# Open-Sentra/beatrice

Measured on AMD Instinct MI355X. Metric: Mpps + achieved HBM GB/s, device-resident parse+filter, 64B and IMIX, higher is better.
Workload: dtype u8; 1 GPU; C2 frames + filter: 16M x 64B Eth/IPv4/UDP, fixed stride, parse + PacketFilter (udp, 10.x.x.x/8, 1000-2000) + ordered compaction (metric's 64B parse+filter); packets_per_gpu=16777216, packets_total=16777216, parallelism=batch split x1, devices_distinct=1, rehearsal_one_device=False

## Files before the change

beatrice_amd/csrc/bt_context.cpp:

```cpp
#include <sched.h>
#include <sys/syscall.h>
#include <unistd.h>

#include <algorithm>
#include <cctype>
#include <cstdarg>
#include <cstdio>
#include <cstdlib>
#include <cstring>
#include <functional>
#include <mutex>
#include <string>
#include <thread>

#include "bt_ctx.h"
#include "bt_hip_util.h"

using namespace bt;

namespace {

thread_local std::string g_err;

}
// ... 213 lines not shown
uint32_t bt_usable_cpus(void) { return bt::usable_cpus(); }

void bt_destroy(bt_ctx* c) {
    const bt::DeviceRestore keep_device;
    if (!c) return;
    (void)hipSetDevice(c->device);
    (void)hipDeviceSynchronize();
    for (const auto& r : c->host_regs)
        (void)bt::pin_release(reinterpret_cast<const void*>(r.first), r.second);
    c->host_regs.clear();
    release_host_pipe(c);
    if (c->pcap) { bt::pcap_stage_free(c->pcap); c->pcap = nullptr; }
    c->pool.reset();
    release_timing_graph(c);
    release_workspace(c);
    release_dfa_pools(c);
    release_timing(c);
    release_extract_stage(c);
    release_xfer(c);
    release_walk_stages(c);
    if (c->stream) (void)hipStreamDestroy(c->stream);
    delete c;
}

int bt_host_parallel(bt_ctx* c, void (*fn)(void*, uint32_t, uint32_t), void* user) {
    if (!c || !fn) return set_error(BT_E_INVALID_ARGUMENT, "null argument");
    bt::host_parallel(c, [&](unsigned w, unsigned T) { fn(user, w, T); });
    return BT_OK;
}

int bt_stream_create(bt_ctx* c, void** stream) {
    const bt::DeviceRestore keep_device;
    if (!c || !stream) return set_error(BT_E_INVALID_ARGUMENT, "null argument");
    HIP_TRY(hipSetDevice(c->device));
    hipStream_t s = nullptr;
    HIP_TRY(hipStreamCreateWithFlags(&s, hipStreamNonBlocking));
    *stream = s;
    return BT_OK;
}

int bt_stream_synchronize(bt_ctx* c, void* stream) {
    const bt::DeviceRestore keep_device;
    if (!c || !stream) return set_error(BT_E_INVALID_ARGUMENT, "null argument");
    HIP_TRY(hipSetDevice(c->device));
    HIP_TRY(hipStreamSynchronize(reinterpret_cast<hipStream_t>(stream)));
    return BT_OK;
}

int bt_stream_destroy(bt_ctx* c, void* stream) {
    const bt::DeviceRestore keep_device;
    if (!c || !stream) return set_error(BT_E_INVALID_ARGUMENT, "null argument");
    HIP_TRY(hipSetDevice(c->device));
    HIP_TRY(hipStreamSynchronize(reinterpret_cast<hipStream_t>(stream)));
    HIP_TRY(hipStreamDestroy(reinterpret_cast<hipStream_t>(stream)));
    return BT_OK;
}

int bt_synchronize(bt_ctx* c) {
    const bt::DeviceRestore keep_device;
    if (!c) return set_error(BT_E_INVALID_ARGUMENT, "null context");
    HIP_TRY(hipSetDevice(c->device));
    HIP_TRY(hipStreamSynchronize(c->stream));
    if (c->ws.cstream) HIP_TRY(hipStreamSynchronize(c->ws.cstream));
    return BT_OK;
}

}

namespace bt {

int ctx_device(const bt_ctx* c) { return c->device; }

bool ctx_stream_busy(bt_ctx* c) {
    const bt::DeviceRestore keep_device;
    if (hipSetDevice(c->device) != hipSuccess) return false;
    return hipStreamQuery(c->stream) == hipErrorNotReady;
}

}
```

beatrice_amd/csrc/bt_ctx.h:

```cpp
#pragma once

#include <hip/hip_runtime.h>
#include <sched.h>

#include <atomic>
#include <chrono>
#include <cstdlib>
#include <memory>
#include <mutex>
#include <utility>
#include <vector>

#include "beatrice_gpu_bench.h"
#include "bt_device.h"
#include "bt_pack.h"
#include "bt_tally.h"
#include "bt_fanout.h"
#include "bt_flowtab.h"
#include "bt_host_pool.h"
#include "bt_host.h"

#define HIP_TRY(x)                                                                       \
    do {                                                                                 \
        hipError_t e_ = (x);                                                             \
// ... 17 lines not shown
    uint8_t* d_in = nullptr;
    uint8_t* h_out = nullptr;
    uint8_t* d_out = nullptr;
    uint32_t* d_tile = nullptr;
    bool busy = false;
    uint32_t lo = 0, cnt = 0;
};

struct PcapStage;
void pcap_stage_free(PcapStage* s);

}

struct bt_ctx {
    int device = 0;
    hipStream_t stream = nullptr;
    bt_opts opts{};
    int grid = 0;
    std::mutex mu;
    int spin_rc = -1;
    unsigned device_flags = 0;

    std::vector<bt_filter_slot> slots;
    bt::DevProgram prog{};
    std::vector<uint8_t> dfa_pool;
    std::atomic<uint32_t> staged_window[2] = {{0u}, {0u}};
    struct DfaPools {
        uint8_t* dev[2] = {nullptr, nullptr};
        std::vector<std::pair<hipStream_t, hipEvent_t>> readers[2];
        std::vector<hipEvent_t> spare;
        int cur = 0;
    } dfa;

    struct Ws {
        uint32_t* chunk_sums = nullptr;
        uint64_t* verdict = nullptr;
        bt::PackChunkSum* pack_sums = nullptr;
        bt::TallyPartial* tally_parts = nullptr;
        uint8_t* fan_parts = nullptr;
        uint8_t* fan_queue = nullptr;
        hipStream_t last = nullptr;
        bool lazy = false;
        hipEvent_t sync = nullptr;
    };
    static constexpr int kMainDone = 8;
    struct Workspace {
        uint32_t cap = 0;
        Ws buf[2];
        int next = 0;
        hipEvent_t main_done[kMainDone] = {};
        int md_next = 0;
        hipStream_t cstream = nullptr;
    } ws;
    const void* last_base = nullptr;
    bool last_base_host = false;

    struct WalkStage {
        bt::RingBlock* h = nullptr;
        uint32_t cap = 0;
        hipEvent_t done = nullptr;
        bool used = false;
    };
    struct WalkStages {
        WalkStage stage[2];
        int next = 0;
    } walk;

    struct HostPipe {
        uint32_t chunk = 0;
        bt::HostSlot hs[2];
        bool ready = false;
        std::atomic<int> waiters{0};
        uint64_t last_caller = 0;
        uint64_t last_end = 0;
        bool shared_call = false;
    } host;
    std::unique_ptr<bt::HostPool> pool;
    std::once_flag pool_once;
    int numa_node = -1;
    cpu_set_t pin{};
    bool pinned = false;

    struct Timing {
        hipEvent_t ev0 = nullptr, ev1 = nullptr;
        hipEvent_t pipe_done = nullptr;
        hipEvent_t pipe_step = nullptr;
        std::vector<hipEvent_t> tev;
    } timing;
    struct TimingGraph {
        hipGraphExec_t exec = nullptr;
        bt_batch batch{};
        bt_outputs out{};
        uint32_t iters = 0;
    } tgraph;

    std::vector<std::pair<uintptr_t, uint64_t>> host_regs;

    struct Xfer {
        std::mutex mu;
        uint8_t* h[2] = {nullptr, nullptr};
        hipEvent_t ev[2] = {nullptr, nullptr};
        hipEvent_t after = nullptr;
    } xfer;

    struct ExtractStage {
        uint8_t* h = nullptr;
        uint8_t* d = nullptr;
        size_t cap = 0;
    } ex;

    bt::PcapStage* pcap = nullptr;
};

namespace bt {

void release_host_pipe(bt_ctx* c);
void release_timing_graph(bt_ctx* c);
void release_workspace(bt_ctx* c);
void release_dfa_pools(bt_ctx* c);
void release_timing(bt_ctx* c);
void release_extract_stage(bt_ctx* c);
void release_xfer(bt_ctx* c);
void release_walk_stages(bt_ctx* c);

HostPool& pool_of(bt_ctx* c);

int dfa_read_on(bt_ctx* c, hipStream_t st);

int ensure_ws(bt_ctx* c, uint32_t n);
int take_ws(bt_ctx* c, uint32_t n, bt_ctx::Ws** w);
int ws_touch(bt_ctx* c, bt_ctx::Ws* w, hipStream_t s);
int ws_done(bt_ctx* c, bt_ctx::Ws* w, hipStream_t s);
int ensure_cstream(bt_ctx* c);
bool host_resident(bt_ctx* c, const void* base);
int check_bounds(hipStream_t st, hipStream_t cst, const char* what);
int run_device(bt_ctx* c, const bt_batch* b, const bt_outputs* o, hipStream_t st, bool aos,
               hipEvent_t e0, hipEvent_t e1, hipStream_t cst = nullptr, hipEvent_t done = nullptr);
int run_pass_pack(bt_ctx* c, const bt_batch* b, const uint64_t* select, const bt_pack_opts* po,
                  const bt_pack_out* out, hipStream_t st, hipEvent_t e0, hipEvent_t e1);

int run_tally(bt_ctx* c, const uint8_t* decide, uint32_t n, const bt_batch* frames, const void* records, uint32_t n_cap,
              uint32_t flags, bt_tally* out, hipStream_t st, hipEvent_t e0, hipEvent_t e1);

int run_fanout(bt_ctx* c, const bt_batch* frames, const uint64_t* select, const bt_fanout_opts* opts, const bt_fanout_out* out,
               hipStream_t st, hipEvent_t e0, hipEvent_t e1);

int run_flow_table(bt_ctx* c, const bt_batch* frames, const uint64_t* select, const bt_flow_table_opts* opts, void* scratch,
                   uint64_t scratch_bytes, const bt_flow_table_out* out, hipStream_t st, hipEvent_t e0, hipEvent_t e1);

int run_flow_track_update(bt_ctx* c, void* state, const bt_batch* frames, const uint64_t* select, const bt_flow_track_update* upd,
                          void* scratch, uint64_t scratch_bytes, const bt_flow_track_out* out, hipStream_t st, hipEvent_t e0,
                          hipEvent_t e1);

int run_flow_tcp(bt_ctx* c, const bt_batch* frames, const uint32_t* flow_id, uint32_t table_flags, bt_flow_tcp_rec* tcp,
                 uint32_t flow_cap, bt_flow_tcp_result* result, hipStream_t st, hipEvent_t e0, hipEvent_t e1);

int run_flow_track_top(bt_ctx* c, const void* state, const bt_flow_top_opts* opts, const bt_flow_tcp_rec* tcp, void* scratch,
                       uint64_t scratch_bytes, const bt_flow_top_out* out, hipStream_t st, hipEvent_t e0, hipEvent_t e1);

int run_flow_track_hosts(bt_ctx* c, const void* state, const bt_flow_hosts_opts* opts, const bt_flow_tcp_rec* tcp, void* scratch,
                         uint64_t scratch_bytes, const bt_flow_hosts_out* out, hipStream_t st, hipEvent_t e0, hipEvent_t e1);

int build_table(const bt_field_def* f, uint32_t n, ExTable* t, uint64_t* span_out, bool* never);
int run_extract(bt_ctx* c, const bt_batch* b, const ExTable& t, bool never, const bt_extract_out* o, hipStream_t st,
                hipEvent_t e0 = nullptr, hipEvent_t e1 = nullptr);

unsigned pipeline_share(const bt_ctx* c);
void publish_staged_window(bt_ctx* c);

template <class Fn>
void pipeline_run(bt_ctx* c, uint32_t cnt, unsigned T, Fn&& fn) {
// ... 41 lines not shown
```

beatrice_amd/csrc/bt_device.h:

```cpp
#pragma once

#include <stdint.h>

#include "beatrice_gpu.h"
#include "bt_bounds.h"
#include "bt_frames.h"

namespace bt {

struct DevFilter {
    uint32_t kind, a, b, ctl;
    uint32_t mask, lo, span, pad;
};
constexpr uint32_t kSelIp = 0, kSelPort = 1, kSelProto = 2, kSelPbit = 3;
constexpr uint32_t kGateNone = 0, kGateIpv4 = 1, kGateL4 = 2;
constexpr uint32_t kResPred = 0, kResThrow = 1, kResHost = 2;

struct DevProgram {
    uint32_t n;
    uint32_t pad[3];
    DevFilter f[BT_MAX_FILTERS];
};

struct MainArgs : FrameSrc {
    uint32_t n_cap;
    uint8_t* records;
    uint8_t* decide;
    uint64_t* verdict;
    uint32_t blocked;
    uint32_t nt;
    const uint8_t* dfa;
    uint32_t dfa_bytes;
    uint32_t prefixes;
    uint32_t lean;
    uint32_t lean_lo;
};
constexpr uint32_t kLeanPcie = 38;
constexpr uint32_t kLeanLo = 12;

constexpr uint32_t kDfaPoolMax = 16384;

constexpr int kWave = 64;
constexpr int kWavesPerBlock = 4;
constexpr int kBlock = kWave * kWavesPerBlock;
constexpr int kRowDwords = 33;
constexpr int kChunkTiles = 256;
constexpr uint32_t kNeedParse = 102;
constexpr uint32_t kNeedFilter = 38;

enum RecLayout { kRecNone = 0, kRecPlanes = 1, kRecAoS = 2, kRecTiled = 3 };
int launch_main(const MainArgs& a, const DevProgram& prog, int rec_layout, bool filter,
                int grid_blocks, bool prefetch, void* stream, void* timing_start = nullptr,
                void* timing_stop = nullptr);
int launch_compact(const uint64_t* verdict, uint32_t n, uint32_t* chunk_sums, uint32_t* pass_idx,
                   uint32_t* n_pass, void* stream);

struct ResumeArgs : FrameSrc {
    uint8_t* decide;
    const uint8_t* dfa;
    uint32_t dfa_bytes;
};
int launch_payload_resume(const ResumeArgs& a, const DevProgram& prog, void* stream, void* timing_start = nullptr,
                          void* timing_stop = nullptr);
int launch_verdict_words(const uint8_t* decide, uint32_t n, uint64_t* verdict, void* stream);
uint32_t bounds_take_resume(void* stream, BoundsLog* first);

inline uint64_t read_limit(const void* base, uint64_t bytes) {
    const uint64_t b = (uint64_t)(uintptr_t)base;
    return bytes ? ((b + bytes + 15u) & ~15ull) - b : 0u;
}

uint32_t bounds_take_main(void* stream, BoundsLog* first);
uint32_t bounds_take_extract(void* stream, BoundsLog* first);

struct RingBlock {
    uint32_t block;
    uint32_t n;
    uint32_t start;
    uint32_t first_off;
};
struct RingWalkArgs {
    const uint8_t* ring;
    uint64_t block_size;
    const RingBlock* blocks;
    uint32_t count;
    bt_pkt_desc* desc;
    uint32_t cap;
    uint32_t* bad;
};
int launch_ring_walk(const RingWalkArgs& a, void* stream);
uint32_t bounds_take_ring(void* stream, BoundsLog* first);

constexpr uint32_t kExWindow = 256;
struct ExField {
    uint32_t offset, length;
    uint32_t ctl;
    uint32_t pad;
};
struct ExTable {
    uint32_t n;
    uint32_t span;
    uint32_t window;
    uint32_t row_dw;
    ExField f[BT_FIELD_MAX];
};
struct ExArgs : FrameSrc {
// ... 14 lines not shown
```

beatrice_amd/csrc/bt_kernels.hip:

```cpp
#include <algorithm>
#include <cstdlib>
#include <type_traits>

#include "bt_dev_util.h"
#include "bt_device.h"
#include "bt_hip_launch.h"
#include "bt_payload_walk.h"
#include "bt_slot_eval.h"

namespace bt {

__device__ BoundsLog g_bounds_main;

namespace {

__device__ __forceinline__ uint32_t be32_of(const uint32_t* w, int i) {
    return (byte_of(w, i) << 24) | (byte_of(w, i + 1) << 16) | (byte_of(w, i + 2) << 8) | byte_of(w, i + 3);
}

__device__ __forceinline__ bool is_vlan(uint32_t et) { return et == 0x8100u || et == 0x88A8u; }

__device__ __forceinline__ uint4 ld16(const uint8_t* p, bool nt) {
    if (nt) {
        const u32x4 x = __builtin_nontemporal_load(reinterpret_cast<const u32x4*>(p));
        return make_uint4(x.x, x.y, x.z, x.w);
    }
    return *reinterpret_cast<const uint4*>(p);
}
__device__ __forceinline__ void st16(uint4* p, uint4 v, bool nt) {
    if (nt) {
        const u32x4 x = {v.x, v.y, v.z, v.w};
        __builtin_nontemporal_store(x, reinterpret_cast<u32x4*>(p));
    } else {
        *p = v;
    }
}

struct Parsed {
    uint32_t r[24];
};

__device__ __forceinline__ uint32_t detect_word(const uint32_t* w0, uint32_t len) {
    const uint32_t et = be16_of(w0, 12), b0 = byte_of(w0, 0), pr = byte_of(w0, 23);
    const uint32_t ports = be16_of(w0, 34) | (be16_of(w0, 36) << 16);
    const bool eth = (len >= 14) & ((et == 0x0800u) | (et == 0x86DDu) | (et == 0x0806u));
    const bool l34 = len >= 34;
    const uint32_t code0 = len < 14 ? BT_DET_UNKNOWN : eth ? BT_DET_ETHERNET : BT_DET_NONE;
    const uint32_t l4code = pr == 6 ? BT_DET_TCP : pr == 17 ? BT_DET_UDP : pr == 1 ? BT_DET_ICMP : 0u;
    const uint32_t code = (eth & l34 & (l4code != 0u)) ? l4code : code0;
    const bool v4 = l34 & ((b0 >> 4) == 4u);
    const bool tcp = v4 & (pr == 6), udp = v4 & (pr == 17);
    const bool p80 = ((ports & 0xFFFFu) == 80u) | ((ports >> 16) == 80u);
    const bool p53 = ((ports & 0xFFFFu) == 53u) | ((ports >> 16) == 53u);
    const uint32_t is = (eth ? BT_IS_ETHERNET : 0u) | (v4 ? BT_IS_IPV4 : 0u) |
                        (((len >= 54) & ((b0 >> 4) == 6u)) ? BT_IS_IPV6 : 0u) | (tcp ? BT_IS_TCP : 0u) |
                        (udp ? BT_IS_UDP : 0u) | ((v4 & (pr == 1)) ? BT_IS_ICMP : 0u) |
                        ((tcp & (len >= 54) & p80) ? BT_IS_HTTP : 0u) | ((udp & (len >= 42) & p53) ? BT_IS_DNS : 0u);
    const uint32_t is2 = (((len >= 28) & (et == 0x0806u)) ? BT_IS2_ARP : 0u) |
                         ((l34 & (pr == 6)) ? BT_IS2_MULTI_TCP : 0u) | ((l34 & (pr == 17)) ? BT_IS2_MULTI_UDP : 0u);
    return code | (is << 8) | (is2 << 16);
}
// ... 396 lines not shown
__device__ __forceinline__ bool round_b(const MainArgs& a, uint32_t t, uint32_t lane, const uint64_t* qa0,
                                       uint32_t* img, const uint32_t* row, uint32_t s, uint64_t my_off,
                                       uint32_t my_len, bool live, bool this_wide, uint32_t need_max,
                                       uint32_t* w0) {
    const uint32_t a_end = this_wide ? round_a_end_wide(my_off & ~15ull, s, my_len, need_max)
                                     : min(64u, s + min(my_len, a.lean));
    const bool cov = a_end >= s + min(my_len, 28u);
    const uint32_t end = !live ? 0u
                       : cov ? s + header_end(w0, my_len, kNeedFilter)
                             : s + min(my_len, need_max);
    const uint32_t lo = (a_end + 15u) >> 4;
    const bool my_nb = end > 16u * lo;
    if (__ballot(my_nb) != 0ull) {
        const bool second = __ballot(my_nb && lo < 4u && end > 16u * (lo + 4u)) != 0ull;
        load_round_b<-1>(a, t, lane, qa0, my_nb ? (lo | (end << 8)) : 0u, img, second);
        wave_lds_sync();
        window<10>(row, s, w0);
    }
    bool wide = __popcll(__ballot(end > 64u)) > 32;
    if (a.nt & 12u) wide = (a.nt & 8u) != 0u;
    return wide;
}

constexpr uint32_t kOob = 0x80000000u;
__device__ __forceinline__ __amdgpu_buffer_rsrc_t rsrc_of(const void* p, uint32_t bytes) {
    return __builtin_amdgcn_make_buffer_rsrc(const_cast<void*>(p), (short)0, (int)bytes, 0x00020000);
}

constexpr bool main_variant(int fixed_log2, int rec, int filter, bool prefetch) {
    return (rec != kRecNone || filter != 0) && (!prefetch || (fixed_log2 < 0 && filter != 2));
}
constexpr bool pipe_variant(int rec, int filter, int dw) {
    return (rec == kRecTiled || (rec == kRecNone && filter != 0)) && filter != 2 && (dw == 1 || dw == 2);
}

constexpr bool late_issue(int fixed_log2, int rec, int filter) {
    return fixed_log2 >= 0 && rec != kRecAoS && filter == 1;
}

constexpr int main_waves_per_eu(int fixed_log2, int rec, int filter) {
    return fixed_log2 < 0 && filter == 2 && rec != kRecAoS ? 4 : 1;
}

struct TileRange {
    uint32_t t, t_end, step;
};
__device__ __forceinline__ TileRange tile_range(const MainArgs& a, uint32_t wid) {
    const uint32_t total_waves = gridDim.x * kWavesPerBlock;
    const uint32_t gw = blockIdx.x * kWavesPerBlock + wid;
    if (a.blocked) {
        const uint32_t per = (a.ntiles + total_waves - 1) / total_waves;
        return {gw * per, min(a.ntiles, gw * per + per), 1u};
    }
    return {gw, a.ntiles, total_waves};
}

__device__ __forceinline__ void store_counted(const MainArgs& a, uint32_t t, uint32_t p0, uint32_t lane, uint32_t code,
                                              uint32_t slot, uint64_t pass) {
    const uint32_t cnt = min(64u, a.n - p0);
    const auto rd = rsrc_of(a.decide ? a.decide + p0 : nullptr, a.decide ? cnt : 0u);
    __builtin_amdgcn_raw_buffer_store_b8((uint8_t)((code << 6) | slot), rd, (int)lane, 0, 0);
    const bool v_in = BT_IN(&g_bounds_main, kSiteVerdict, t, a.ntiles);
    const auto rv = rsrc_of(a.verdict ? a.verdict + t : nullptr, a.verdict && v_in ? 8u : 0u);
    const u32x2 pv = {(uint32_t)pass, (uint32_t)(pass >> 32)};
    __builtin_amdgcn_raw_buffer_store_b64(pv, rv, lane == 0 ? 0 : (int)kOob, 0, 0);
}

template <int FIXED_LOG2, int REC, int FILTER, bool PREFETCH>
__global__ __launch_bounds__(kBlock) __attribute__((amdgpu_waves_per_eu(main_waves_per_eu(FIXED_LOG2, REC, FILTER))))
void bt_parse_filter_main(MainArgs a, DevProgram prog) {
    static_assert(main_variant(FIXED_LOG2, REC, FILTER, PREFETCH), "a variant launch_t never launches");
    constexpr uint32_t kRow = row_dw<FIXED_LOG2>();
    constexpr uint32_t kImg = REC == kRecAoS && kRow < BT_REC_BYTES / 4 ? kWave * (BT_REC_BYTES / 4) : kWave * kRow;
    __shared__ __attribute__((aligned(16))) uint32_t lds_all[kWavesPerBlock * kImg + 32];
    extern __shared__ uint4 dyn_lds[];
    const uint32_t lane = threadIdx.x & 63u;
    const uint32_t wid = __builtin_amdgcn_readfirstlane(threadIdx.x >> 6);
    uint32_t* img = lds_all + wid * kImg;
    const uint32_t* row = img + lane * kRow;
    if (FILTER == 2 && a.dfa_bytes) copy_dfa_pool(dyn_lds, a.dfa, a.dfa_bytes, &g_bounds_main);
    const uint8_t* dfa_lds = reinterpret_cast<const uint8_t*>(dyn_lds);

    const TileRange tiles = tile_range(a, wid);
    const uint32_t t_end = tiles.t_end, step = tiles.step;
    uint32_t t = tiles.t;
    const uint32_t need_max = REC != kRecNone ? kNeedParse : kNeedFilter;
    const HotProgram hot = hot_program(prog);
    bool wide = false;
    Stage<FIXED_LOG2> st;
    constexpr bool LATE = late_issue(FIXED_LOG2, REC, FILTER);
    if ((PREFETCH || LATE) && t < t_end) issue_loads<FIXED_LOG2, LATE>(a, t, lane, st, wide, need_max);
    if (LATE && t < t_end) {
        const auto r = rsrc_of(g_zero16, 0u);
        __builtin_amdgcn_raw_buffer_store_b8((uint8_t)0, r, 0, 0, 0);
        const u32x2 z = {0u, 0u};
        __builtin_amdgcn_raw_buffer_store_b64(z, r, 16, 0, 0);
    }
    for (; t < t_end; t += step) {
        const uint32_t p0 = t * 64u;
        const uint32_t my = p0 + lane;
        const bool live = my < a.n;

        if (!PREFETCH && !LATE) issue_loads<FIXED_LOG2>(a, t, lane, st, wide, need_max);
        stage_to_lds<FIXED_LOG2>(st, img, lane);
        const uint64_t my_off = st.off;
        const uint32_t my_len = st.len;
        uint64_t qa0[FIXED_LOG2 >= 0 ? 1 : 4];
#pragma unroll
        for (int j = 0; j < (FIXED_LOG2 >= 0 ? 1 : 4); ++j) qa0[j] = st.qa0[j];
        wave_lds_sync();
        const bool this_wide = FIXED_LOG2 < 0 && st.wide;
        if (PREFETCH && t + step < t_end) issue_loads<FIXED_LOG2>(a, t + step, lane, st, wide, need_max);
        const uint32_t s = (FIXED_LOG2 >= 0) ? 0u : ((uint32_t)my_off & 15u);
        uint32_t w0[10];
        window<10>(row, s, w0);
        if constexpr (FIXED_LOG2 < 0) {
            if (REC != kRecNone)
                wide = round_b(a, t, lane, qa0, img, row, s, my_off, my_len, live, this_wide, need_max, w0);
        }

        const uint32_t len = live ? my_len : 0u;

        if (REC != kRecNone && live) {
            Parsed p;
            if (REC == kRecPlanes || REC == kRecTiled) {
                const uint32_t ns = parse_packet<true>(row, s, len, w0, p);
                if (REC == kRecTiled) {
                    uint4* tile = reinterpret_cast<uint4*>(a.records) + (uint64_t)t * (BT_REC_SLABS * 64);
                    const uint64_t below = (1ull << lane) - 1ull;
                    const bool rec_in = BT_IN(&g_bounds_main, kSiteRecord, t, (a.n_cap + 63u) / 64u);
#pragma unroll
                    for (uint32_t k = 0; k < BT_REC_SLABS; ++k) {
                        const uint64_t mk = __ballot(k < ns);
                        if (mk == 0ull) break;
                        if (k < ns && rec_in)
                            st16(tile + k * 64 + (k < 2u ? lane : (uint32_t)__popcll(mk & below)),
                                 make_uint4(p.r[4 * k], p.r[4 * k + 1], p.r[4 * k + 2], p.r[4 * k + 3]), a.nt & 1u);
                    }
                } else {
                    uint4* dst = reinterpret_cast<uint4*>(a.records) + (uint64_t)my;
#pragma unroll
                    for (uint32_t k = 0; k < BT_REC_SLABS; ++k)
                        if ((k < 2u || __ballot(k < ns) != 0ull) && BT_IN(&g_bounds_main, kSiteRecord, my, a.n_cap))
                            st16(dst + (uint64_t)k * a.n_cap,
                                 make_uint4(p.r[4 * k], p.r[4 * k + 1], p.r[4 * k + 2], p.r[4 * k + 3]), a.nt & 1u);
                }
            }
        }
        Parsed aos;
        if (REC == kRecAoS) {
            parse_packet<false>(row, s, len, w0, aos);
            if (!live)
#pragma unroll
                for (int k = 0; k < 24; ++k) aos.r[k] = 0u;
        }

        if (REC == kRecTiled && !live) {
            uint4* tile = reinterpret_cast<uint4*>(a.records) + (uint64_t)t * (BT_REC_SLABS * 64);
            if (BT_IN(&g_bounds_main, kSiteRecord, t, (a.n_cap + 63u) / 64u)) {
                st16(tile + lane, make_uint4(0, 0, 0, 0), a.nt & 1u);
                st16(tile + 64 + lane, make_uint4(0, 0, 0, 0), a.nt & 1u);
            }
        }

        if (LATE && t + step < t_end) issue_loads<FIXED_LOG2, LATE>(a, t + step, lane, st, wide, need_max);
        if (FILTER) {
            uint32_t slot;
            const uint32_t reuse = FIXED_LOG2 < 0 && a.lean == 0xFFFFu && !this_wide ? 4u : 0u;
            const uint32_t code = filter_packet<FILTER>(a, prog, hot, dfa_lds, img + lane * kRow, kRow, my_off, len, w0, live,
                                                        slot, reuse);
            const uint64_t pass = __ballot(live && code == BT_DECIDE_PASS);
            if (LATE) {
                store_counted(a, t, p0, lane, code, slot, pass);
            } else {
                if (a.decide && live && BT_IN(&g_bounds_main, kSiteDecide, my, a.n)) a.decide[my] = (uint8_t)((code << 6) | slot);
                if (lane == 0 && a.verdict && BT_IN(&g_bounds_main, kSiteVerdict, t, a.ntiles))
                    a.verdict[t] = pass;
            }
        }
        if (REC == kRecAoS) {
            wave_lds_sync();
            uint4* lrec = reinterpret_cast<uint4*>(img);
#pragma unroll
            for (uint32_t k = 0; k < BT_REC_SLABS; ++k)
                lrec[lane * BT_REC_SLABS + k] = make_uint4(aos.r[4 * k], aos.r[4 * k + 1], aos.r[4 * k + 2], aos.r[4 * k + 3]);
            wave_lds_sync();
            const uint32_t q_end = min(64u, a.n - p0) * BT_REC_SLABS;
            uint4* dst = reinterpret_cast<uint4*>(a.records + (uint64_t)p0 * BT_REC_BYTES);
#pragma unroll
            for (uint32_t i = 0; i < BT_REC_SLABS; ++i) {
                const uint32_t q = i * 64u + lane;
                if (q < q_end && BT_IN(&g_bounds_main, kSiteRecord, (uint64_t)p0 * BT_REC_SLABS + q,
                                       (uint64_t)a.n_cap * BT_REC_SLABS))
                    st16(dst + q, lrec[q], a.nt & 1u);
            }
        }
        wave_lds_sync();
    }
}



#ifndef BT_DESC_AUX
#define BT_DESC_AUX 0
#endif
#ifndef BT_DESC_AUX_Q
#define BT_DESC_AUX_Q 2
#endif
template <int DW>
struct TileDesc {
    uint32_t me[DW + 1];
    uint32_t q[4][DW + 1];
};

template <int DW>
__device__ __forceinline__ void load_desc_pipe(const MainArgs& a, uint32_t t, bool valid, uint32_t lane,
                                               TileDesc<DW>& d) {
    const uint32_t p0 = t * 64u;
    const uint32_t cnt = valid && p0 < a.n ? min(64u, a.n - p0) : 0u;
    const auto r = rsrc_of(a.desc + (valid ? (uint64_t)DW * p0 : 0ull), cnt * 8u * DW);
    const uint32_t qoff = (lane >> 2) * 8u * DW;
    if constexpr (DW == 1) {
        const u32x2 v = __builtin_amdgcn_raw_buffer_load_b64(r, (int)(lane * 8u), 0, BT_DESC_AUX);
        d.me[0] = v.x; d.me[1] = v.y;
#pragma unroll
        for (uint32_t j = 0; j < 4; ++j) {
            const u32x2 w = __builtin_amdgcn_raw_buffer_load_b64(r, (int)(qoff + j * 128u), 0, BT_DESC_AUX_Q);
            d.q[j][0] = w.x; d.q[j][1] = w.y;
        }
    } else {
        typedef unsigned int u32x3 __attribute__((ext_vector_type(3)));
        const u32x3 v = __builtin_amdgcn_raw_buffer_load_b96(r, (int)(lane * 16u), 0, BT_DESC_AUX);
        d.me[0] = v.x; d.me[1] = v.y; d.me[2] = v.z;
#pragma unroll
        for (uint32_t j = 0; j < 4; ++j) {
            const u32x3 w = __builtin_amdgcn_raw_buffer_load_b96(r, (int)(qoff + j * 256u), 0, BT_DESC_AUX_Q);
            d.q[j][0] = w.x; d.q[j][1] = w.y; d.q[j][2] = w.z;
        }
    }
}

template <int DW>
__device__ __forceinline__ void decode_desc(const uint32_t (&w)[DW + 1], uint64_t& off, uint32_t& len) {
    const uint64_t d = ((uint64_t)w[1] << 32) | w[0];
    if constexpr (DW == 1) desc_packed(d, off, len);
    else desc_xdp(d, w[2], off, len);
}

template <int DW>
__device__ __forceinline__ void issue_round_a_pipe(const MainArgs& a, uint32_t lane, const TileDesc<DW>& d,
// ... 147 lines not shown
    const uint64_t word = t < ntiles ? verdict[t] : 0ull;

    uint32_t pre = 0, tot = 0;
    for (uint32_t i = tid; i < nchunks; i += 256) {
        const uint32_t x = chunk_sums[i];
        tot += x;
        if (i < c) pre += x;
    }
    for (int o = 32; o > 0; o >>= 1) { pre += __shfl_xor(pre, o); tot += __shfl_xor(tot, o); }
    if (lane == 0) { red[wid] = pre; wsum[wid] = tot; }
    __syncthreads();
    const uint32_t base = red[0] + red[1] + red[2] + red[3];
    if (c == 0 && tid == 0 && n_pass) *n_pass = wsum[0] + wsum[1] + wsum[2] + wsum[3];
    if (!pass_idx) return;
    __syncthreads();

    const uint32_t v = (uint32_t)__popcll(word);
    uint32_t incl = v;
    for (int o = 1; o < 64; o <<= 1) {
        const uint32_t y = __shfl_up(incl, o);
        if (lane >= (uint32_t)o) incl += y;
    }
    if (lane == 63) red[wid] = incl;
    words[tid] = word;
    __syncthreads();
    uint32_t wpre = 0;
    for (uint32_t w = 0; w < wid; ++w) wpre += red[w];
    tile_off[tid] = base + wpre + incl - v;
    __syncthreads();

    const uint64_t below_mask = (1ull << lane) - 1ull;
    const uint32_t first = wid * 64u;
    for (uint32_t i = 0; i < 64u; i += 4u) {
        uint64_t w4[4];
        uint32_t o4[4];
#pragma unroll
        for (uint32_t k = 0; k < 4u; ++k) { w4[k] = words[first + i + k]; o4[k] = tile_off[first + i + k]; }
#pragma unroll
        for (uint32_t k = 0; k < 4u; ++k)
            if (((w4[k] >> lane) & 1ull) &&
                BT_IN(&g_bounds_main, kSitePassIdx, o4[k] + (uint32_t)__popcll(w4[k] & below_mask), n))
                pass_idx[o4[k] + (uint32_t)__popcll(w4[k] & below_mask)] = (c * kChunkTiles + first + i + k) * 64u + lane;
    }
}

bool use_pipe() {
    static const bool on = [] {
        const char* e = getenv("BT_NO_PIPE");
        return !(e && *e && *e != '0');
    }();
    return on;
}

template <auto Kernel>
void launch_variant(const MainArgs& a, const DevProgram& prog, int grid, int auto_grid, int cap_per_cu, uint32_t dyn,
                    hipStream_t st, hipEvent_t e0, hipEvent_t e1) {
    const uint32_t needed = (a.ntiles + kWavesPerBlock - 1) / kWavesPerBlock;
    int g = grid;
    if (g <= 0) {
        g = auto_grid > 0 ? auto_grid : resident_grid<Kernel>(dyn);
        if (cap_per_cu) g = std::min(g, cap_per_cu * cu_count());
    }
    if ((uint32_t)g > needed) g = (int)(needed ? needed : 1);
    launch(Kernel, dim3(g), dim3(kBlock), dyn, st, e0, e1, a, prog);
}

template <int FL, int REC, int F>
void launch_t(const MainArgs& a, const DevProgram& prog, int grid, bool pf, hipStream_t st, hipEvent_t e0,
              hipEvent_t e1) {
    const uint32_t dyn = F == 2 ? (a.dfa_bytes + 15u) & ~15u : 0u;
    if constexpr (FL < 0 && pipe_variant(REC, F, 1) && pipe_variant(REC, F, 2)) {
        if (pf && a.desc && (a.nt & 1u) && use_pipe()) {
            if (a.desc_words == 1) launch_variant<bt_parse_filter_pipe<REC, F, 1>>(a, prog, grid, 0, 2, dyn, st, e0, e1);
            else launch_variant<bt_parse_filter_pipe<REC, F, 2>>(a, prog, grid, 0, 2, dyn, st, e0, e1);
            return;
        }
    }
    if constexpr (main_variant(FL, REC, F, true)) {
        if (pf) {
            launch_variant<bt_parse_filter_main<FL, REC, F, true>>(a, prog, grid, 0, 0, dyn, st, e0, e1);
            return;
        }
    }
    if constexpr (FL < 0 && F == 2) {
        static const int pay_grid = [] {
            const char* e = getenv("BT_PAYLOAD_GRID");
            return e && *e ? atoi(e) : -3;
        }();
        const uint32_t needed = (a.ntiles + kWavesPerBlock - 1) / kWavesPerBlock;
        const int per = pay_grid < 0 ? (int)((needed + (uint32_t)(-pay_grid) - 1u) / (uint32_t)(-pay_grid)) : 0;
        launch_variant<bt_parse_filter_main<FL, REC, F, false>>(a, prog, grid, per, std::max(pay_grid, 0), dyn, st, e0, e1);
        return;
    }
    constexpr int cap = FL < 0 ? 0 : F && !late_issue(FL, REC, F) ? 3 : 2;
    launch_variant<bt_parse_filter_main<FL, REC, F, false>>(a, prog, grid, 0, cap, dyn, st, e0, e1);
}

template <int FL>
void launch_fl(const MainArgs& a, const DevProgram& prog, int rec, int f, int grid, bool pf, hipStream_t st,
               hipEvent_t e0, hipEvent_t e1) {
    auto by_f = [&](auto rec_c) {
        constexpr int R = decltype(rec_c)::value;
        if (f == 2) launch_t<FL, R, 2>(a, prog, grid, pf, st, e0, e1);
        else if (f == 1) launch_t<FL, R, 1>(a, prog, grid, pf, st, e0, e1);
        else launch_t<FL, R, 0>(a, prog, grid, pf, st, e0, e1);
    };
    if (rec == kRecPlanes) by_f(std::integral_constant<int, kRecPlanes>{});
    else if (rec == kRecTiled) by_f(std::integral_constant<int, kRecTiled>{});
    else if (rec == kRecAoS) by_f(std::integral_constant<int, kRecAoS>{});
    else if (f == 2) launch_t<FL, kRecNone, 2>(a, prog, grid, pf, st, e0, e1);
    else launch_t<FL, kRecNone, 1>(a, prog, grid, pf, st, e0, e1);
}

}

int launch_main(const MainArgs& a, const DevProgram& prog, int rec_layout, bool filter, int grid_blocks,
                bool prefetch, void* stream, void* timing_start, void* timing_stop) {
    hipStream_t st = reinterpret_cast<hipStream_t>(stream);
    hipEvent_t e0 = reinterpret_cast<hipEvent_t>(timing_start), e1 = reinterpret_cast<hipEvent_t>(timing_stop);
    const int grid = grid_blocks;
    int fl = -1;
    if (!a.desc) {
        if (a.stride == 16) fl = 0;
        else if (a.stride == 32) fl = 1;
        else if (a.stride == 64) fl = 2;
        else if (a.stride == 128) fl = 3;
    }
    const int f = !filter ? 0 : a.dfa_bytes ? 2 : 1;
    switch (fl) {
    case 0: launch_fl<0>(a, prog, rec_layout, f, grid, prefetch, st, e0, e1); break;
    case 1: launch_fl<1>(a, prog, rec_layout, f, grid, prefetch, st, e0, e1); break;
    case 2: launch_fl<2>(a, prog, rec_layout, f, grid, prefetch, st, e0, e1); break;
    case 3: launch_fl<3>(a, prog, rec_layout, f, grid, prefetch, st, e0, e1); break;
    default: launch_fl<-1>(a, prog, rec_layout, f, grid, prefetch, st, e0, e1); break;
    }
    return hipGetLastError() == hipSuccess ? BT_OK : BT_E_INTERNAL;
}

int launch_compact(const uint64_t* verdict, uint32_t n, uint32_t* chunk_sums, uint32_t* pass_idx,
                   uint32_t* n_pass, void* stream) {
    hipStream_t st = reinterpret_cast<hipStream_t>(stream);
    const uint32_t ntiles = (n + 63u) / 64u;
    const uint32_t nchunks = (ntiles + kChunkTiles - 1) / kChunkTiles;
    if (nchunks == 0) return BT_OK;
    hipLaunchKernelGGL(bt_chunk_sums, dim3(nchunks), dim3(256), 0, st, verdict, ntiles, chunk_sums, nchunks);
    hipLaunchKernelGGL(bt_compact, dim3(nchunks), dim3(256), 0, st, verdict, chunk_sums, nchunks, ntiles, n, pass_idx,
                       n_pass);
    return hipGetLastError() == hipSuccess ? BT_OK : BT_E_INTERNAL;
}

uint32_t bounds_take_main(void* stream, BoundsLog* first) { return bounds_take(g_bounds_main, stream, first); }

}
```

beatrice_amd/csrc/bt_launch.cpp:

```cpp
#include <algorithm>
#include <cstdio>
#include <cstdlib>
#include <mutex>

#include "bt_ctx.h"
#include "bt_hip_util.h"
#include "bt_resume_host.h"

using namespace bt;

namespace {

void free_ws(bt_ctx* c) {
    for (auto& w : c->ws.buf) {
        if (w.chunk_sums) (void)hipFree(w.chunk_sums);
        if (w.verdict) (void)hipFree(w.verdict);
        if (w.pack_sums) (void)hipFree(w.pack_sums);
        if (w.tally_parts) (void)hipFree(w.tally_parts);
        if (w.fan_parts) (void)hipFree(w.fan_parts);
        if (w.fan_queue) (void)hipFree(w.fan_queue);
        w.fan_parts = nullptr;
        w.fan_queue = nullptr;
        w.pack_sums = nullptr;
        w.tally_parts = nullptr;
        w.chunk_sums = nullptr; w.verdict = nullptr; w.last = nullptr; w.lazy = false;
    }
    c->ws.cap = 0;
}

bool ctx_stream(const bt_ctx* c, hipStream_t s) { return s == c->stream || (c->ws.cstream && s == c->ws.cstream); }

}

namespace bt {

int ensure_ws(bt_ctx* c, uint32_t n) {
    if (n <= c->ws.cap && c->ws.buf[0].chunk_sums) return BT_OK;
    HIP_TRY(hipSetDevice(c->device));
    if (c->tgraph.exec) { (void)hipGraphExecDestroy(c->tgraph.exec); c->tgraph.exec = nullptr; }
    if (c->ws.buf[0].chunk_sums) HIP_TRY(hipDeviceSynchronize());
    free_ws(c);
    const uint32_t ntiles = (std::max(n, 1u) + 63) / 64;
    const uint32_t nchunks = (ntiles + kChunkTiles - 1) / kChunkTiles;
    for (auto& w : c->ws.buf) {
        if (!w.sync) HIP_TRY(hipEventCreateWithFlags(&w.sync, hipEventDisableTiming));
        HIP_TRY(hipMalloc(&w.chunk_sums, (size_t)nchunks * 4));
        HIP_TRY(hipMalloc(&w.verdict, (size_t)ntiles * 8));
        HIP_TRY(hipMalloc(&w.pack_sums, (size_t)nchunks * sizeof(PackChunkSum) + (size_t)ntiles * 4));
        HIP_TRY(hipMalloc(&w.tally_parts, (size_t)nchunks * sizeof(TallyPartial)));
        HIP_TRY(hipMalloc(&w.fan_parts, fan_ws_bytes(nchunks)));
        HIP_TRY(hipMalloc(&w.fan_queue, (size_t)ntiles * 64));
    }
    for (auto& e : c->ws.main_done)
        if (!e) HIP_TRY(hipEventCreateWithFlags(&e, hipEventDisableTiming));
    c->ws.cap = ntiles * 64;
    return BT_OK;
}

int take_ws(bt_ctx* c, uint32_t n, bt_ctx::Ws** w) {
    if (int rc = ensure_ws(c, n)) return rc;
    *w = &c->ws.buf[c->ws.next];
    c->ws.next ^= 1;
    return BT_OK;
}

int ws_touch(bt_ctx* c, bt_ctx::Ws* w, hipStream_t s) {
    if (w->last && w->last != s) {
        if (w->lazy) HIP_TRY(hipEventRecord(w->sync, w->last));
        HIP_TRY(hipStreamWaitEvent(s, w->sync, 0));
    }
    (void)c;
    return BT_OK;
}

int ws_done(bt_ctx* c, bt_ctx::Ws* w, hipStream_t s) {
    w->last = s;
    w->lazy = ctx_stream(c, s);
    if (!w->lazy) HIP_TRY(hipEventRecord(w->sync, s));
    return BT_OK;
}
// ... 60 lines not shown
        if (done) HIP_TRY(hipEventRecord(done, st));
        return BT_OK;
    }
    bt_ctx::Ws* w = nullptr;
    if (int rc = compact ? take_ws(c, b->n, &w) : BT_OK) return rc;
    if (bad) return set_error(BT_E_INVALID_ARGUMENT, "%s", why);
    if ((b->flags & BT_BATCH_LEAN) && o->records)
        return set_error(BT_E_INVALID_ARGUMENT, "a BT_BATCH_LEAN batch holds frame bytes 12..43 only: no records");
    a.bytes = read_limit(a.base, a.bytes);
    a.prefixes = (b->flags & (BT_BATCH_PREFIXES | BT_BATCH_LEAN)) ? 1u : 0u;
    a.n_cap = o->records ? o->n_cap : 0;
    a.records = reinterpret_cast<uint8_t*>(o->records);
    a.decide = o->decide;
    a.verdict = o->verdict ? o->verdict : (w ? w->verdict : nullptr);
    if (w && !o->verdict) { int rc = ws_touch(c, w, st); if (rc) return rc; }
    a.blocked = (c->opts.flags & BT_OPT_TILE_BLOCKED) ? 1u : 0u;
    a.lean = 0xFFFFu;
    const bool lean = b->desc && !o->records && !(c->opts.flags & BT_OPT_NO_LEAN_PCIE) && host_resident(c, b->base);
    a.dfa = c->dfa.dev[c->dfa.cur];
    a.dfa_bytes = filter ? (uint32_t)c->dfa_pool.size() : 0u;
    if (c->opts.flags & BT_OPT_CACHE_DEFAULT) a.nt = 0;
    else a.nt = 3u;
    if (a.dfa_bytes && !(c->opts.flags & BT_OPT_NT_LOADS)) a.nt &= ~2u;
    if (c->opts.flags & BT_OPT_NT_STORES) a.nt |= 1u;
    if (c->opts.flags & BT_OPT_NT_LOADS) a.nt |= 2u;
    if (c->opts.flags & BT_OPT_WIDE_NEVER) a.nt |= 4u;
    if (c->opts.flags & BT_OPT_WIDE_ALWAYS) a.nt |= 8u;
    a.lean_lo = 0;
    if (lean && !(a.nt & 8u)) {
        static const uint32_t lean_end = [] {
            const char* e = getenv("BT_LEAN_END");
            return e && atoi(e) >= (int)kNeedFilter ? (uint32_t)atoi(e) : kLeanPcie;
        }();
        static const uint32_t lean_lo = [] {
            const char* e = getenv("BT_LEAN_LO");
            return e && atoi(e) >= 0 && atoi(e) <= 12 ? (uint32_t)atoi(e) : kLeanLo;
        }();
        a.lean = lean_end;
        a.lean_lo = lean_lo;
        a.nt |= 4u;
    }
    int rec = kRecNone;
    if (o->records) {
        if (aos || (c->opts.flags & BT_OPT_RECORDS_AOS)) rec = kRecAoS;
        else if (c->opts.flags & BT_OPT_RECORDS_PLANES) rec = kRecPlanes;
        else rec = kRecTiled;
    }
    const bool piped = compact && cst != st;
    hipEvent_t mend = e1;
    if (piped && !e1) {
        mend = c->ws.main_done[c->ws.md_next];
        c->ws.md_next = (c->ws.md_next + 1) % bt_ctx::kMainDone;
    }
    int rc = launch_main(a, c->prog, rec, filter, c->grid, !(c->opts.flags & BT_OPT_NO_PREFETCH), st, e0, mend);
    if (rc) return set_error(rc, "main kernel launch failed: %s", hipGetErrorString(hipGetLastError()));
    if (w && !o->verdict) { if ((rc = ws_done(c, w, st))) return rc; }
    if (a.dfa_bytes && (rc = dfa_read_on(c, st))) return rc;
    if (compact) {
        if (piped) HIP_TRY(hipStreamWaitEvent(cst, mend, 0));
        if ((rc = ws_touch(c, w, cst))) return rc;
        rc = launch_compact(a.verdict, b->n, w->chunk_sums, o->pass_idx, o->n_pass, cst);
        if (rc) return set_error(rc, "compaction launch failed");
        if ((rc = ws_done(c, w, cst))) return rc;
        if (done) HIP_TRY(hipEventRecord(done, cst));
    } else if (done) {
        HIP_TRY(hipEventRecord(done, st));
    }
    return check_bounds(st, cst, "parse+filter");
}

int run_pass_pack(bt_ctx* c, const bt_batch* b, const uint64_t* select, const bt_pack_opts* po,
                  const bt_pack_out* out, hipStream_t st, hipEvent_t e0, hipEvent_t e1) {
    if (!c || !b || !select || !po || !out || !out->total || !out->n_packed)
        return set_error(BT_E_INVALID_ARGUMENT, "null argument");
    if (!out->bytes && out->cap) return set_error(BT_E_INVALID_ARGUMENT, "null output with cap %llu", (unsigned long long)out->cap);
    if (b->flags & (BT_BATCH_PREFIXES | BT_BATCH_LEAN))
        return set_error(BT_E_INVALID_ARGUMENT, "a BT_BATCH_PREFIXES / BT_BATCH_LEAN batch holds no whole frames to pack");
    if (po->lead > kPackLeadMax) return set_error(BT_E_INVALID_ARGUMENT, "lead %u > %u", po->lead, kPackLeadMax);
    if (po->align != 1 && po->align != 16 && po->align != 64)
        return set_error(BT_E_INVALID_ARGUMENT, "align %u (1, 16 or 64)", po->align);
    PackArgs a{};
    char why[128];
    if (frame_src(b, &a, why, sizeof(why))) return set_error(BT_E_INVALID_ARGUMENT, "%s", why);
    HIP_TRY(hipSetDevice(c->device));
    if (b->n == 0) {
        HIP_TRY(hipMemsetAsync(out->total, 0, 8, st));
        HIP_TRY(hipMemsetAsync(out->n_packed, 0, 4, st));
        return BT_OK;
    }
    bt_ctx::Ws* w = nullptr;
    int rc = take_ws(c, b->n, &w);
    if (rc) return rc;
    if ((rc = ws_touch(c, w, st))) return rc;
    a.nchunks = (a.ntiles + kPackChunkTiles - 1) / kPackChunkTiles;
    a.lead = po->lead;
    a.snap = po->snap;
    a.align = po->align;
    a.select = select;
    a.out = out->bytes;
    a.cap = out->cap;
    a.out_desc = out->desc;
    a.total = out->total;
    a.n_packed = out->n_packed;
    a.sums = w->pack_sums;
    rc = launch_pass_pack(a, st, e0, e1);
    if (rc) return set_error(rc, "pack kernel launch failed: %s", hipGetErrorString(hipGetLastError()));
    return ws_done(c, w, st);
}

void ctx_forget_base(bt_ctx* c) {
    std::lock_guard<std::mutex> lk(c->mu);
    c->last_base = nullptr;
}

void release_workspace(bt_ctx* c) {
    free_ws(c);
    for (auto& w : c->ws.buf)
        if (w.sync) (void)hipEventDestroy(w.sync);
    for (auto e : c->ws.main_done)
        if (e) (void)hipEventDestroy(e);
    if (c->ws.cstream) (void)hipStreamDestroy(c->ws.cstream);
}

void release_walk_stages(bt_ctx* c) {
    for (auto& w : c->walk.stage) {
        if (w.h) (void)hipHostFree(w.h);
        if (w.done) (void)hipEventDestroy(w.done);
    }
}

}

extern "C" {

int bt_reserve(bt_ctx* c, uint32_t n) {
    const bt::DeviceRestore keep_device;
    if (!c) return set_error(BT_E_INVALID_ARGUMENT, "null context");
    std::lock_guard<std::mutex> lk(c->mu);
    return ensure_ws(c, n);
}

int bt_parse_filter_device(bt_ctx* c, const bt_batch* b, const bt_outputs* o, void* stream) {
    const bt::DeviceRestore keep_device;
    if (!c) return set_error(BT_E_INVALID_ARGUMENT, "null context");
    std::lock_guard<std::mutex> lk(c->mu);
    hipStream_t st = stream ? reinterpret_cast<hipStream_t>(stream) : c->stream;
    return run_device(c, b, o, st, false, nullptr, nullptr);
}

int bt_filter_resume_device(bt_ctx* c, const bt_batch* b, const bt_outputs* o, void* stream) {
    const bt::DeviceRestore keep_device;
    ResumeArgs a{};
    if (const char* why = resume_args_error(c, b, o, &a)) return set_error(BT_E_INVALID_ARGUMENT, "%s", why);
    std::lock_guard<std::mutex> lk(c->mu);
    hipStream_t st = stream ? reinterpret_cast<hipStream_t>(stream) : c->stream;
    HIP_TRY(hipSetDevice(c->device));
    const bool compact = o->pass_idx || o->n_pass;
    if (b->n == 0) {
        if (o->n_pass) HIP_TRY(hipMemsetAsync(o->n_pass, 0, 4, st));
        return BT_OK;
    }
    a.bytes = read_limit(a.base, a.bytes);
    a.decide = o->decide;
    a.dfa = c->dfa.dev[c->dfa.cur];
    a.dfa_bytes = (uint32_t)c->dfa_pool.size();
    int rc = launch_payload_resume(a, c->prog, st);
    if (rc) return set_error(rc, "resume kernel launch failed: %s", hipGetErrorString(hipGetLastError()));
    if (a.dfa_bytes && (rc = dfa_read_on(c, st))) return rc;
    if (o->verdict || compact) {
        bt_ctx::Ws* w = nullptr;
        if (compact) {
            if ((rc = take_ws(c, b->n, &w))) return rc;
            if ((rc = ws_touch(c, w, st))) return rc;
        }
// ... 93 lines not shown
```

Baseline: 50150 Mpps.

## Add dynamic atomic work-stealing for the tail tiles of the main parse+filter kernel

The fixed-stride filter kernel now processes most tiles with static grid-stride assignment and leaves the last few rounds as a tail. Waves claim that tail through relaxed atomic tickets spread over 8 sharded head counters, with claims issued one step ahead to hide latency. The aim is to cut imbalance at the end of the kernel, where some waves finish early while others still work. In exchange it adds a per-stream counter buffer that uses double-buffered sets reset by block 0, some atomic traffic, extra control flow in the hot loop, and stream bookkeeping plus cleanup on stream destroy.

Result: faster. 51630 Mpps, median of 6 (+2.9%).

```diff
diff --git a/beatrice_amd/csrc/bt_context.cpp b/beatrice_amd/csrc/bt_context.cpp
--- a/beatrice_amd/csrc/bt_context.cpp
+++ b/beatrice_amd/csrc/bt_context.cpp
@@ -289,6 +289,10 @@
     if (!c || !stream) return set_error(BT_E_INVALID_ARGUMENT, "null argument");
     HIP_TRY(hipSetDevice(c->device));
     HIP_TRY(hipStreamSynchronize(reinterpret_cast<hipStream_t>(stream)));
+    {
+        std::lock_guard<std::mutex> lk(c->mu);
+        bt::forget_stream(c, reinterpret_cast<hipStream_t>(stream));
+    }
     HIP_TRY(hipStreamDestroy(reinterpret_cast<hipStream_t>(stream)));
     return BT_OK;
 }
diff --git a/beatrice_amd/csrc/bt_ctx.h b/beatrice_amd/csrc/bt_ctx.h
--- a/beatrice_amd/csrc/bt_ctx.h
+++ b/beatrice_amd/csrc/bt_ctx.h
@@ -93,6 +93,13 @@
         int md_next = 0;
         hipStream_t cstream = nullptr;
     } ws;
+    struct TailHeads {
+        hipStream_t stream = nullptr;
+        uint32_t* dev = nullptr;
+        uint32_t launches = 0;
+    };
+    static constexpr size_t kTailStreams = 64;
+    std::vector<TailHeads> tail;
     const void* last_base = nullptr;
     bool last_base_host = false;
 
@@ -158,6 +165,7 @@
 void release_host_pipe(bt_ctx* c);
 void release_timing_graph(bt_ctx* c);
 void release_workspace(bt_ctx* c);
+void forget_stream(bt_ctx* c, hipStream_t st);
 void release_dfa_pools(bt_ctx* c);
 void release_timing(bt_ctx* c);
 void release_extract_stage(bt_ctx* c);
diff --git a/beatrice_amd/csrc/bt_device.h b/beatrice_amd/csrc/bt_device.h
--- a/beatrice_amd/csrc/bt_device.h
+++ b/beatrice_amd/csrc/bt_device.h
@@ -34,6 +34,12 @@
     uint32_t prefixes;
     uint32_t lean;
     uint32_t lean_lo;
+    uint32_t* tail_heads;
+    uint32_t tail_set;
+    uint32_t tail_static;
+    uint32_t tail_claim;
+    uint32_t tail_visits;
+    uint32_t tail_stride;
 };
 constexpr uint32_t kLeanPcie = 38;
 constexpr uint32_t kLeanLo = 12;
@@ -52,6 +58,7 @@
 int launch_main(const MainArgs& a, const DevProgram& prog, int rec_layout, bool filter,
                 int grid_blocks, bool prefetch, void* stream, void* timing_start = nullptr,
                 void* timing_stop = nullptr);
+bool main_deals_tail(const MainArgs& a, int rec_layout, bool filter);
 int launch_compact(const uint64_t* verdict, uint32_t n, uint32_t* chunk_sums, uint32_t* pass_idx,
                    uint32_t* n_pass, void* stream);
 
diff --git a/beatrice_amd/csrc/bt_kernels.hip b/beatrice_amd/csrc/bt_kernels.hip
--- a/beatrice_amd/csrc/bt_kernels.hip
+++ b/beatrice_amd/csrc/bt_kernels.hip
@@ -1,4 +1,5 @@
 #include <algorithm>
+#include <cstdio>
 #include <cstdlib>
 #include <type_traits>
 
@@ -7,6 +8,7 @@
 #include "bt_hip_launch.h"
 #include "bt_payload_walk.h"
 #include "bt_slot_eval.h"
+#include "bt_tail_split.h"
 
 namespace bt {
 
@@ -509,7 +511,7 @@
         const uint32_t per = (a.ntiles + total_waves - 1) / total_waves;
         return {gw * per, min(a.ntiles, gw * per + per), 1u};
     }
-    return {gw, a.ntiles, total_waves};
+    return {gw, a.tail_heads ? a.tail_static : a.ntiles, total_waves};
 }
 
 __device__ __forceinline__ void store_counted(const MainArgs& a, uint32_t t, uint32_t p0, uint32_t lane, uint32_t code,
@@ -546,20 +548,71 @@
     bool wide = false;
     Stage<FIXED_LOG2> st;
     constexpr bool LATE = late_issue(FIXED_LOG2, REC, FILTER);
-    if ((PREFETCH || LATE) && t < t_end) issue_loads<FIXED_LOG2, LATE>(a, t, lane, st, wide, need_max);
-    if (LATE && t < t_end) {
+    const bool dyn = LATE && a.tail_heads != nullptr && !a.blocked;
+    const TailSplit split = {a.tail_static, a.tail_claim};
+    const TailShape shape = tail_shape(a.ntiles, split);
+    uint32_t head = blockIdx.x & (kTailHeads - 1u);
+    uint32_t heads_left = gridDim.x >= kTailHeads ? a.tail_visits : kTailHeads;
+    uint32_t lim = t_end, stride = step;
+    uint32_t next_unit = kNoTile;
+    uint32_t ahead = 0u;
+    bool ahead_out = false;
+    auto take = [&]() -> uint32_t {
+        uint32_t k = 0u;
+        if (lane == 0)
+            k = __hip_atomic_fetch_add(a.tail_heads + (a.tail_set * kTailHeads + head) * a.tail_stride, 1u, __ATOMIC_RELAXED,
+                                       __HIP_MEMORY_SCOPE_AGENT);
+        return k;
+    };
+    auto read = [&](uint32_t k) -> uint32_t {
+        const uint32_t u = ticket_unit(shape, head, __builtin_amdgcn_readfirstlane(k));
+        if (u == kNoTile) { head = (head + 1u) & (kTailHeads - 1u); --heads_left; }
+        return u;
+    };
+    auto next_tile = [&](uint32_t cur) -> uint32_t {
+        uint32_t tn = cur + stride;
+        if (cur == kNoTile || tn >= lim) {
+            if (!dyn) return kNoTile;
+            uint32_t u = next_unit;
+            next_unit = kNoTile;
+            while (u == kNoTile && heads_left) u = read(take());
+            if (u == kNoTile) return kNoTile;
+            tn = unit_first(split, u);
+            stride = shape.units;
+            lim = unit_limit(a.ntiles, split, shape, u);
+        }
+        if (dyn && tn + stride >= lim && heads_left) {
+            ahead = take();
+            ahead_out = true;
+        }
+        return tn;
+    };
+    auto after_wait = [&]() {
+        if (dyn && ahead_out) {
+            next_unit = read(ahead);
+            ahead_out = false;
+        }
+    };
+    if (dyn && blockIdx.x == 0 && wid == 0 && lane < kTailHeads)
+        __hip_atomic_store(a.tail_heads + ((a.tail_set ^ 1u) * kTailHeads + lane) * a.tail_stride, 0u, __ATOMIC_RELAXED,
+                           __HIP_MEMORY_SCOPE_AGENT);
+    if (dyn && t >= t_end) t = next_tile(kNoTile);
+    const bool any = dyn ? t != kNoTile : t < t_end;
+    if ((PREFETCH || LATE) && any) issue_loads<FIXED_LOG2, LATE>(a, t, lane, st, wide, need_max);
+    if (LATE && any) {
         const auto r = rsrc_of(g_zero16, 0u);
         __builtin_amdgcn_raw_buffer_store_b8((uint8_t)0, r, 0, 0, 0);
         const u32x2 z = {0u, 0u};
         __builtin_amdgcn_raw_buffer_store_b64(z, r, 16, 0, 0);
     }
-    for (; t < t_end; t += step) {
+    auto tile = [&](const uint32_t t, auto&& waited, auto&& next) __attribute__((always_inline)) {
         const uint32_t p0 = t * 64u;
         const uint32_t my = p0 + lane;
         const bool live = my < a.n;
 
         if (!PREFETCH && !LATE) issue_loads<FIXED_LOG2>(a, t, lane, st, wide, need_max);
         stage_to_lds<FIXED_LOG2>(st, img, lane);
+        waited();
         const uint64_t my_off = st.off;
         const uint32_t my_len = st.len;
         uint64_t qa0[FIXED_LOG2 >= 0 ? 1 : 4];
@@ -620,7 +673,10 @@
             }
         }
 
-        if (LATE && t + step < t_end) issue_loads<FIXED_LOG2, LATE>(a, t + step, lane, st, wide, need_max);
+        if constexpr (LATE) {
+            const uint32_t tn = next();
+            if (tn != kNoTile) issue_loads<FIXED_LOG2, LATE>(a, tn, lane, st, wide, need_max);
+        }
         if (FILTER) {
             uint32_t slot;
             const uint32_t reuse = FIXED_LOG2 < 0 && a.lean == 0xFFFFu && !this_wide ? 4u : 0u;
@@ -653,6 +709,19 @@
             }
         }
         wave_lds_sync();
+    };
+    const uint32_t s_end = !dyn ? t_end : t_end > 2u * step ? t_end - 2u * step : 0u;
+    if (!dyn || lim == t_end)
+        for (; t < s_end; t += step)
+            tile(t, [] {}, [&] { return t + step < t_end ? t + step : kNoTile; });
+    if constexpr (LATE) {
+        if (dyn) {
+            while (t != kNoTile) {
+                uint32_t tn = kNoTile;
+                tile(t, after_wait, [&] { return tn = next_tile(t); });
+                t = tn;
+            }
+        }
     }
 }
 
@@ -906,7 +975,26 @@
     return on;
 }
 
-template <auto Kernel>
+struct TailKnob {
+    uint32_t rounds, claim, visits, stride;
+};
+const TailKnob& tail_knob() {
+    static const TailKnob k = [] {
+        TailKnob v{kTailRounds, kTailClaim, kTailVisits, kTailStride};
+        if (const char* e = getenv("BT_TAIL")) {
+            unsigned r = 0, c = 0, h = 0, s = 0;
+            const int got = sscanf(e, "%u,%u,%u,%u", &r, &c, &h, &s);
+            if (got >= 1) v.rounds = r;
+            if (got >= 2 && c) v.claim = c;
+            if (got >= 3 && h >= 1 && h <= kTailHeads) v.visits = h;
+            if (got >= 4 && s >= 1 && s <= kTailStride) v.stride = s;
+        }
+        return v;
+    }();
+    return k;
+}
+
+template <auto Kernel, bool TAIL = false>
 void launch_variant(const MainArgs& a, const DevProgram& prog, int grid, int auto_grid, int cap_per_cu, uint32_t dyn,
                     hipStream_t st, hipEvent_t e0, hipEvent_t e1) {
     const uint32_t needed = (a.ntiles + kWavesPerBlock - 1) / kWavesPerBlock;
@@ -916,7 +1004,16 @@
         if (cap_per_cu) g = std::min(g, cap_per_cu * cu_count());
     }
     if ((uint32_t)g > needed) g = (int)(needed ? needed : 1);
-    launch(Kernel, dim3(g), dim3(kBlock), dyn, st, e0, e1, a, prog);
+    MainArgs b = a;
+    if (!TAIL || a.blocked || tail_knob().rounds == 0u) b.tail_heads = nullptr;
+    if (b.tail_heads) {
+        const TailSplit s = tail_split(a.ntiles, (uint32_t)g * kWavesPerBlock, tail_knob().rounds, tail_knob().claim);
+        b.tail_static = s.n_static;
+        b.tail_claim = s.claim;
+        b.tail_visits = tail_knob().visits;
+        b.tail_stride = tail_knob().stride;
+    }
+    launch(Kernel, dim3(g), dim3(kBlock), dyn, st, e0, e1, b, prog);
 }
 
 template <int FL, int REC, int F>
@@ -947,7 +1044,7 @@
         return;
     }
     constexpr int cap = FL < 0 ? 0 : F && !late_issue(FL, REC, F) ? 3 : 2;
-    launch_variant<bt_parse_filter_main<FL, REC, F, false>>(a, prog, grid, 0, cap, dyn, st, e0, e1);
+    launch_variant<bt_parse_filter_main<FL, REC, F, false>, late_issue(FL, REC, F)>(a, prog, grid, 0, cap, dyn, st, e0, e1);
 }
 
 template <int FL>
@@ -968,6 +1065,11 @@
 
 }
 
+bool main_deals_tail(const MainArgs& a, int rec_layout, bool filter) {
+    const bool fixed = !a.desc && (a.stride == 16 || a.stride == 32 || a.stride == 64 || a.stride == 128);
+    return fixed && filter && !a.dfa_bytes && rec_layout != kRecAoS && !a.blocked && tail_knob().rounds != 0u;
+}
+
 int launch_main(const MainArgs& a, const DevProgram& prog, int rec_layout, bool filter, int grid_blocks,
                 bool prefetch, void* stream, void* timing_start, void* timing_stop) {
     hipStream_t st = reinterpret_cast<hipStream_t>(stream);
diff --git a/beatrice_amd/csrc/bt_launch.cpp b/beatrice_amd/csrc/bt_launch.cpp
--- a/beatrice_amd/csrc/bt_launch.cpp
+++ b/beatrice_amd/csrc/bt_launch.cpp
@@ -6,6 +6,7 @@
 #include "bt_ctx.h"
 #include "bt_hip_util.h"
 #include "bt_resume_host.h"
+#include "bt_tail_split.h"
 
 using namespace bt;
 
@@ -26,6 +27,26 @@
         w.chunk_sums = nullptr; w.verdict = nullptr; w.last = nullptr; w.lazy = false;
     }
     c->ws.cap = 0;
+}
+
+bt_ctx::TailHeads* tail_heads_for(bt_ctx* c, hipStream_t st) {
+    hipStreamCaptureStatus cs = hipStreamCaptureStatusNone;
+    if (hipStreamIsCapturing(st, &cs) != hipSuccess || cs != hipStreamCaptureStatusNone) {
+        (void)hipGetLastError();
+        return nullptr;
+    }
+    for (auto& t : c->tail)
+        if (t.stream == st) return &t;
+    if (c->tail.size() >= bt_ctx::kTailStreams) return nullptr;
+    uint32_t* d = nullptr;
+    if (hipMalloc(&d, kTailWords * sizeof(uint32_t)) != hipSuccess ||
+        hipMemsetAsync(d, 0, kTailWords * sizeof(uint32_t), st) != hipSuccess) {
+        (void)hipGetLastError();
+        if (d) (void)hipFree(d);
+        return nullptr;
+    }
+    c->tail.push_back({st, d, 0u});
+    return &c->tail.back();
 }
 
 bool ctx_stream(const bt_ctx* c, hipStream_t s) { return s == c->stream || (c->ws.cstream && s == c->ws.cstream); }
@@ -192,6 +213,11 @@
         mend = c->ws.main_done[c->ws.md_next];
         c->ws.md_next = (c->ws.md_next + 1) % bt_ctx::kMainDone;
     }
+    if (main_deals_tail(a, rec, filter))
+        if (bt_ctx::TailHeads* t = tail_heads_for(c, st)) {
+            a.tail_heads = t->dev;
+            a.tail_set = t->launches++ & 1u;
+        }
     int rc = launch_main(a, c->prog, rec, filter, c->grid, !(c->opts.flags & BT_OPT_NO_PREFETCH), st, e0, mend);
     if (rc) return set_error(rc, "main kernel launch failed: %s", hipGetErrorString(hipGetLastError()));
     if (w && !o->verdict) { if ((rc = ws_done(c, w, st))) return rc; }
@@ -260,6 +286,17 @@
     for (auto e : c->ws.main_done)
         if (e) (void)hipEventDestroy(e);
     if (c->ws.cstream) (void)hipStreamDestroy(c->ws.cstream);
+    for (auto& t : c->tail) (void)hipFree(t.dev);
+    c->tail.clear();
+}
+
+void forget_stream(bt_ctx* c, hipStream_t st) {
+    for (size_t i = 0; i < c->tail.size(); ++i)
+        if (c->tail[i].stream == st) {
+            (void)hipFree(c->tail[i].dev);
+            c->tail.erase(c->tail.begin() + (long)i);
+            return;
+        }
 }
 
 void release_walk_stages(bt_ctx* c) {
diff --git a/beatrice_amd/csrc/bt_tail_split.h b/beatrice_amd/csrc/bt_tail_split.h
--- /dev/null
+++ b/beatrice_amd/csrc/bt_tail_split.h
@@ -0,0 +1,63 @@
+#pragma once
+
+#include <stdint.h>
+
+#ifdef __HIPCC__
+#define BT_TAIL_HD __host__ __device__
+#else
+#define BT_TAIL_HD
+#endif
+
+namespace bt {
+
+constexpr uint32_t kTailHeads = 8;
+constexpr uint32_t kTailStride = 1024;
+constexpr uint32_t kTailWords = 2 * kTailHeads * kTailStride;
+constexpr uint32_t kNoTile = 0xFFFFFFFFu;
+
+#ifndef BT_TAIL_ROUNDS
+#define BT_TAIL_ROUNDS 8
+#endif
+#ifndef BT_TAIL_CLAIM
+#define BT_TAIL_CLAIM 2
+#endif
+constexpr uint32_t kTailRounds = BT_TAIL_ROUNDS;
+constexpr uint32_t kTailClaim = BT_TAIL_CLAIM;
+constexpr uint32_t kTailVisits = 2;
+
+struct TailSplit {
+    uint32_t n_static;
+    uint32_t claim;
+};
+
+BT_TAIL_HD inline TailSplit tail_split(uint32_t ntiles, uint32_t total_waves, uint32_t rounds = kTailRounds,
+                                       uint32_t claim = kTailClaim) {
+    const uint32_t w = total_waves ? total_waves : 1u;
+    const uint32_t full = ntiles / w;
+    return {full > rounds ? (full - rounds) * w : 0u, claim ? claim : 1u};
+}
+
+struct TailShape {
+    uint32_t tail;
+    uint32_t units;
+    uint32_t per_head;
+};
+BT_TAIL_HD inline TailShape tail_shape(uint32_t ntiles, TailSplit s) {
+    const uint32_t tail = ntiles - s.n_static;
+    const uint32_t units = (tail + s.claim - 1u) / s.claim;
+    return {tail, units, (units + kTailHeads - 1u) / kTailHeads};
+}
+BT_TAIL_HD inline uint32_t head_units(TailShape sh, uint32_t head) {
+    const uint32_t first = head * sh.per_head;
+    return first >= sh.units ? 0u : (sh.units - first < sh.per_head ? sh.units - first : sh.per_head);
+}
+BT_TAIL_HD inline uint32_t ticket_unit(TailShape sh, uint32_t head, uint32_t k) {
+    return k < head_units(sh, head) ? head * sh.per_head + k : kNoTile;
+}
+BT_TAIL_HD inline uint32_t unit_first(TailSplit s, uint32_t unit) { return s.n_static + unit; }
+BT_TAIL_HD inline uint32_t unit_limit(uint32_t ntiles, TailSplit s, TailShape sh, uint32_t unit) {
+    const uint64_t lim = (uint64_t)s.n_static + unit + (uint64_t)s.claim * sh.units;
+    return lim < ntiles ? (uint32_t)lim : ntiles;
+}
+
+}
```
